# tturturiello/lightweight-snappy

Measured on AMD Instinct MI355X. Metric: compress + decompress MB/s at 1/2/4/8 MI355X; % HBM roofline; ratio vs ref, higher is better.
Workload: dtype u8

## Files before the change

### lightweight-snappy_amd/csrc/snappy_k2_emit.inc

```
    __shared__ __attribute__((aligned(16))) uint8_t stage_[kK2Stage + 4 + 4 * 64 + 16];
    auto *const stage = (__attribute__((address_space(3))) uint8_t *)stage_;
    const uint32_t lane = threadIdx.x;
    const uint32_t u = blockIdx.x;
    const uint32_t nt = ntok[u];
#if K2_RECORDS
    const uint64_t base = 0;
    const uint32_t L = rec.L;
#else
    const uint64_t base = (uint64_t)u * unit;
    const uint32_t L = (uint32_t)((n - base) < unit ? (n - base) : unit);
#endif
    const uint8_t *src = in + base;
    uint8_t *dst = out + offsets[u];
#if K2_RECORDS
    const uint32_t *tok = rec.tok, *tok_full = rec.tok_full;
#else
    const uint32_t *tok = reinterpret_cast<const uint32_t *>(tokens) + (uint64_t)u * tok_cap;
    const uint32_t *tok_full = reinterpret_cast<const uint32_t *>(tokens) + ((uint64_t)gridDim.x + u) * tok_cap;
#endif
    if (blockIdx.y == 0) {
        if (hdr_mode == SNAPPY_HDR_EVERY_UNIT) varint_put(L, dst, lane);
        else if (hdr_mode == SNAPPY_HDR_FIRST_UNIT && (K2_RECORDS || u == 0)) varint_put(header_value, dst, lane);
    }
    uint32_t kwn[kK2Per];
    auto load_kw = [&](uint32_t c, uint32_t *k) {
#pragma unroll
        for (uint32_t i = 0; i < kK2Per; i++) {
            const uint32_t t = c + kK2Per * lane + i;
            k[i] = tok[t < nt ? t : 0u];
        }
    };
    auto load_se = [&](uint32_t sg) {
#if K2_RECORDS
        return *reinterpret_cast<const uint2 *>(rec.segu + 2 * (sg * kK2Seg <= nt ? sg : 0u));
#else
        return *reinterpret_cast<const uint2 *>(seg_off + 2 * ((uint64_t)u * segs + (sg * kK2Seg <= nt ? sg : 0u)));
#endif
    };
    if (blockIdx.y * kK2Seg <= nt) load_kw(blockIdx.y * kK2Seg, kwn);
    uint2 sen = load_se(blockIdx.y);
    for (uint32_t sg = blockIdx.y; sg * kK2Seg <= nt; sg += gridDim.y) {
    const uint2 se = sen;
    sen = load_se(sg + gridDim.y);
    uint32_t o = se.x, carry = se.y;
    for (uint32_t c = sg * kK2Seg; c < (sg + 1) * kK2Seg && c <= nt; c += kK2Pass) {

    uint32_t gap[kK2Per], len[kK2Per], off[kK2Per], pe[kK2Per], litn[kK2Per], hl[kK2Per], sz[kK2Per];
    bool live[kK2Per];
    uint32_t lspan = 0;
    uint32_t kw[kK2Per];
#pragma unroll
    for (uint32_t i = 0; i < kK2Per; i++) kw[i] = kwn[i];
    {
        uint32_t cn = c + kK2Pass;
        if (!(cn < (sg + 1) * kK2Seg && cn <= nt)) cn = (sg + gridDim.y) * kK2Seg;
        if (cn <= nt) load_kw(cn, kwn);
    }
#pragma unroll
    for (uint32_t i = 0; i < kK2Per; i++) {
        const uint32_t t = c + kK2Per * lane + i;
        const bool has = t < nt;
        live[i] = t <= nt;
        const uint32_t k = has ? kw[i] : 0xFFFFFFFFu;
        const uint32_t lc = (k >> 16) & 0xFF, gc = k >> 24;
        off[i] = has ? k & 0xFFFF : 0u;
        gap[i] = has ? gc : 0u;
        len[i] = has ? lc + 4 : 0u;
        if (has && (lc == 255 || gc == 255)) {
            const uint32_t f = tok_full[t];
            gap[i] = f & 0xFFFF;
            len[i] = f >> 16;
        }
        lspan += gap[i] + len[i];
    }
    uint32_t span_tot;
    uint32_t cur = carry + wave_excl_scan(lspan, lane, &span_tot);
    uint32_t lsum = 0;
#pragma unroll
    for (uint32_t i = 0; i < kK2Per; i++) {
        const uint32_t t = c + kK2Per * lane + i;
        pe[i] = cur;
        litn[i] = t < nt ? gap[i] : (t == nt ? L - cur : 0u);
        cur += gap[i] + len[i];
        hl[i] = litn[i] ? (litn[i] <= 60 ? 1 : (litn[i] <= 256 ? 2 : 3)) : 0;
        sz[i] = hl[i] + litn[i] + ((live[i] && len[i]) ? copy_bytes(len[i], off[i]) : 0);
        lsum += sz[i];
    }
    uint32_t total;
    uint32_t rel = wave_excl_scan(lsum, lane, &total);
    const bool staged = total <= kK2Stage;
    const uint32_t sb = staged ? (uint32_t)(reinterpret_cast<uintptr_t>(dst + o) & 3) : 0u;
    uint64_t longs[kK2Per];
    uint32_t d0v[kK2Per];
    uint32_t lw[kK2Per][5], lsh[kK2Per];
    bool wide[kK2Per];
#pragma unroll
    for (uint32_t i = 0; i < kK2Per; i++) {
        wide[i] = base + pe[i] + 20 <= n;
        const bool ld = !SNAPPY_K2_NOLIT && staged && wide[i] && live[i] && litn[i] != 0 && litn[i] <= 16;
        const uintptr_t sa = reinterpret_cast<uintptr_t>(src + pe[i]);
        lsh[i] = (uint32_t)(sa & 3);
        const auto *aw = reinterpret_cast<const __attribute__((address_space(1))) uint32_t *>(
            ld ? sa - lsh[i] : reinterpret_cast<uintptr_t>(tok));
#pragma unroll
        for (uint32_t j = 0; j < 5; j++) lw[i][j] = aw[j];
    }
#pragma unroll
    for (uint32_t i = 0; i < kK2Per; i++) {
        const bool wide_ok = wide[i];
        if (staged) put_element_lds(stage, rel + sb, src, pe[i], litn[i], hl[i], len[i], off[i], wide_ok, live[i], lane,
                                    lw[i], lsh[i]);
        else if (live[i]) put_element(dst + o + rel, src, pe[i], litn[i], hl[i], len[i], off[i], wide_ok);
        longs[i] = __ballot(live[i] && litn[i] > 16);
        d0v[i] = rel + sb + hl[i];
        rel += sz[i];
    }
#pragma unroll
    for (uint32_t i = 0; i < kK2Per && !SNAPPY_K2_NOLIT; i++) {
        if (staged) k2_long_literals(stage, src, longs[i], litn[i], pe[i], d0v[i], lane);
        else k2_long_literals(dst + o, src, in + n, longs[i], litn[i], pe[i], d0v[i], lane);
    }
    if (staged) {
        __builtin_amdgcn_wave_barrier();
        uint8_t *g = dst + o;
        uint32_t head = (4 - sb) & 3;
        if (head > total) head = total;
        if (lane < head) g[lane] = stage[sb + lane];
        const uint32_t nw = (total - head) >> 2;
        uint32_t *gw = reinterpret_cast<uint32_t *>(g + head);
        const auto *sw = reinterpret_cast<const __attribute__((address_space(3))) uint32_t *>(stage + sb + head);
        for (uint32_t k = lane; k < nw; k += 64) gw[k] = sw[k];
        const uint32_t tail0 = head + 4 * nw;
        if (lane < total - tail0) g[tail0 + lane] = stage[sb + tail0 + lane];
    }
    __builtin_amdgcn_wave_barrier();
    o += total;
    carry += span_tot;
    }
    }
```

### lightweight-snappy_amd/csrc/snappy_kernels.hip

```cpp
#include <hip/hip_runtime.h>
#include <stdint.h>
#include <type_traits>

#include "snappy_kernels.h"

#ifndef SNAPPY_TU
#define SNAPPY_TU 0
#endif
#define SNAPPY_TU_COMPRESS (SNAPPY_TU != 2)
#define SNAPPY_TU_DECODE (SNAPPY_TU != 1)

#if ((defined(SNAPPY_K2_NOLIT) && SNAPPY_K2_NOLIT) || defined(SNAPPY_K4_NOFAR)) && !defined(SNAPPY_MEASUREMENT_BUILD)
#error "SNAPPY_K2_NOLIT / SNAPPY_K4_NOFAR write wrong output: measurement builds only (-DSNAPPY_MEASUREMENT_BUILD)"
#endif

namespace snappy_amd {

__device__ int amdgcn_writelane(int val, int lanesel, int old) __asm("llvm.amdgcn.writelane.i32");


constexpr uint32_t kTable = 4096;
constexpr uint32_t kMul = 0x1e35a7bdu;

typedef uint32_t u32x4 __attribute__((ext_vector_type(4)));
// ... 1249 lines not shown
    }
#endif
#ifdef SNAPPY_K1R_STATS
    if (!REC && lane == 0) {
        uint64_t *st = reinterpret_cast<uint64_t *>(tokens + (uint64_t)gridDim.x * tok_cap) + 4 * (uint64_t)u;
        st[0] = clock64() - t_loop;
#if defined(SNAPPY_K1R_LSTAMPS)
        st[1] = seg[0] | (seg[1] << 32);
        st[3] = seg[2] | (seg[3] << 32);
        st[2] = seg[4] | (seg[5] << 32);
#else
        st[1] = n_farc | ((uint64_t)n_reload << 32);
        st[2] = n_probe | ((uint64_t)n_round << 32);
        st[3] = n_match | ((uint64_t)n_refresh << 32);
#endif
    }
#endif
}

#if SNAPPY_TU_COMPRESS
__global__ __launch_bounds__(64, 3) void k1r_match_units(const uint8_t *__restrict__ in, uint64_t n, uint32_t unit,
                                                          uint32_t hdr_mode, uint64_t header_value,
                                                          uint2 *__restrict__ tokens, uint32_t tok_cap,
                                                          uint32_t *__restrict__ ntok_out,
                                                          uint32_t *__restrict__ sizes,
                                                          uint32_t *__restrict__ seg_off, uint32_t segs)
{
    k1r_body<false>(in, n, unit, hdr_mode, header_value, tokens, tok_cap, ntok_out, sizes, seg_off, segs);
}
#endif

#if SNAPPY_TU_COMPRESS
__global__ __launch_bounds__(64, 3) void k1r_match_units64(const uint8_t *__restrict__ in, uint64_t n, uint32_t unit,
                                                            uint32_t hdr_mode, uint64_t header_value,
                                                            uint2 *__restrict__ tokens, uint32_t tok_cap,
                                                            uint32_t *__restrict__ ntok_out,
                                                            uint32_t *__restrict__ sizes,
                                                            uint32_t *__restrict__ seg_off, uint32_t segs)
{
    k1r_body<true>(in, n, unit, hdr_mode, header_value, tokens, tok_cap, ntok_out, sizes, seg_off, segs);
}
#endif

__device__ __forceinline__ uint64_t rfl64(uint64_t v)
{
    return ((uint64_t)rfl((uint32_t)(v >> 32)) << 32) | rfl((uint32_t)v);
}

template <bool BIG>
__device__ __forceinline__ void kr1_record(const uint8_t *__restrict__ in, const uint64_t *__restrict__ off_len,
                                           const uint32_t *__restrict__ list, const uint64_t *__restrict__ sbase,
                                           uint32_t *__restrict__ scratch, uint32_t *__restrict__ ntok_out,
                                           uint32_t *__restrict__ sizes)
{
    K1Record rec;
    rec.u = rfl(list[blockIdx.x]);
    rec.L = rfl((uint32_t)off_len[2 * (uint64_t)rec.u + 1]);
    rec.src = in + rfl64(off_len[2 * (uint64_t)rec.u]);
    const uint32_t tok_cap = records_tok_cap(rec.L);
    rec.tok = scratch + rfl64(sbase[rec.u]);
    rec.tok_full = rec.tok + tok_cap;
    rec.segu = rec.tok_full + tok_cap;
    k1r_body<BIG, true>(nullptr, 0, 0, SNAPPY_HDR_EVERY_UNIT, 0, nullptr, 0, ntok_out, sizes, nullptr, 0, rec);
}

#if SNAPPY_TU_COMPRESS
__global__ __launch_bounds__(64, 3) void kr1_match_records(const uint8_t *__restrict__ in,
                                                            const uint64_t *__restrict__ off_len,
                                                            const uint32_t *__restrict__ list,
                                                            const uint64_t *__restrict__ sbase,
                                                            uint32_t *__restrict__ scratch,
                                                            uint32_t *__restrict__ ntok_out,
                                                            uint32_t *__restrict__ sizes)
{
    kr1_record<false>(in, off_len, list, sbase, scratch, ntok_out, sizes);
}

__global__ __launch_bounds__(64, 3) void kr1_match_records64(const uint8_t *__restrict__ in,
                                                              const uint64_t *__restrict__ off_len,
                                                              const uint32_t *__restrict__ list,
                                                              const uint64_t *__restrict__ sbase,
                                                              uint32_t *__restrict__ scratch,
                                                              uint32_t *__restrict__ ntok_out,
                                                              uint32_t *__restrict__ sizes)
{
    kr1_record<true>(in, off_len, list, sbase, scratch, ntok_out, sizes);
}
#endif

template <bool BIG>
__device__ __forceinline__ void kr1_lunit(const uint8_t *__restrict__ in, const uint64_t *__restrict__ off_len,
                                          const uint32_t *__restrict__ list, const uint32_t *__restrict__ urec,
                                          const uint64_t *__restrict__ ubase, const uint64_t *__restrict__ sbase,
                                          uint32_t *__restrict__ scratch, uint32_t *__restrict__ ntok_out,
                                          uint32_t *__restrict__ sizes)
{
    K1Record rec;
    rec.u = rfl(list[blockIdx.x]);
    const uint32_t r = rfl(urec[rec.u]);
    const uint32_t blk = rec.u - rfl((uint32_t)ubase[r]);
    const uint64_t len = rfl64(off_len[2 * (uint64_t)r + 1]);
    const uint64_t at = (uint64_t)blk * SNAPPY_BLOCK;
    rec.L = (uint32_t)(len - at < SNAPPY_BLOCK ? len - at : SNAPPY_BLOCK);
    rec.src = in + rfl64(off_len[2 * (uint64_t)r]) + at;
    const uint32_t tok_cap = records_tok_cap(rec.L);
    rec.tok = scratch + rfl64(sbase[rec.u]);
    rec.tok_full = rec.tok + tok_cap;
    rec.segu = rec.tok_full + tok_cap;
    k1r_body<BIG, true>(nullptr, 0, 0, blk == 0 ? SNAPPY_HDR_FIRST_UNIT : SNAPPY_HDR_NONE, len, nullptr, 0, ntok_out,
                        sizes, nullptr, 0, rec);
}

#if SNAPPY_TU_COMPRESS
__global__ __launch_bounds__(64, 3) void kr1_match_lunits(const uint8_t *__restrict__ in,
                                                           const uint64_t *__restrict__ off_len,
                                                           const uint32_t *__restrict__ list,
                                                           const uint32_t *__restrict__ urec,
                                                           const uint64_t *__restrict__ ubase,
                                                           const uint64_t *__restrict__ sbase,
                                                           uint32_t *__restrict__ scratch,
                                                           uint32_t *__restrict__ ntok_out,
                                                           uint32_t *__restrict__ sizes)
{
    kr1_lunit<false>(in, off_len, list, urec, ubase, sbase, scratch, ntok_out, sizes);
}

__global__ __launch_bounds__(64, 3) void kr1_match_lunits64(const uint8_t *__restrict__ in,
                                                             const uint64_t *__restrict__ off_len,
                                                             const uint32_t *__restrict__ list,
                                                             const uint32_t *__restrict__ urec,
                                                             const uint64_t *__restrict__ ubase,
                                                             const uint64_t *__restrict__ sbase,
                                                             uint32_t *__restrict__ scratch,
                                                             uint32_t *__restrict__ ntok_out,
                                                             uint32_t *__restrict__ sizes)
{
    kr1_lunit<true>(in, off_len, list, urec, ubase, sbase, scratch, ntok_out, sizes);
}
#endif

__device__ __forceinline__ uint32_t wave_excl_scan32(uint32_t v, uint32_t *total)
{
    uint32_t x = v;
    x += dpp0<0x111, 0xF>(x);
    x += dpp0<0x112, 0xF>(x);
    x += dpp0<0x114, 0xF>(x);
    x += dpp0<0x118, 0xF>(x);
    x += dpp0<0x142, 0xA>(x);
    *total = (uint32_t)__builtin_amdgcn_readlane((int)x, 31);
    return x - v;
}

template <typename P>
__device__ __forceinline__ void put_copy(P *o, uint32_t len, uint32_t off)
{
    while (len > 68) {
        o[0] = 0xFE; o[1] = (uint8_t)off; o[2] = (uint8_t)(off >> 8);
        o += 3; len -= 64;
    }
    if (len > 64) {
        o[0] = 0xEE; o[1] = (uint8_t)off; o[2] = (uint8_t)(off >> 8);
        o += 3; len -= 60;
    }
    if (len < 12 && off < 2048) {
        o[0] = (uint8_t)((((off >> 8) << 5) + ((len - 4) << 2) + 1));
        o[1] = (uint8_t)off;
    } else {
        o[0] = (uint8_t)(((len - 1) << 2) | 2); o[1] = (uint8_t)off; o[2] = (uint8_t)(off >> 8);
    }
}

template <typename P>
__device__ __forceinline__ void put_element(P *w, const uint8_t *__restrict__ src, uint32_t s0, uint32_t litn,
                                            uint32_t hl, uint32_t len, uint32_t off, bool wide_ok)
{
    if (hl == 1) w[0] = (uint8_t)((litn - 1) << 2);
    else if (hl == 2) { w[0] = 60 << 2; w[1] = (uint8_t)(litn - 1); }
    else if (hl == 3) { w[0] = 61 << 2; w[1] = (uint8_t)(litn - 1); w[2] = (uint8_t)((litn - 1) >> 8); }
    if (litn <= 16) {
        if (wide_ok) {
            const uintptr_t sa = reinterpret_cast<uintptr_t>(src + s0);
            const uint32_t sh = (uint32_t)(sa & 3);
            const uint32_t *aw = reinterpret_cast<const uint32_t *>(sa - sh);
            const uint32_t d0 = aw[0], d1 = aw[1], d2 = aw[2], d3 = aw[3], d4 = aw[4];
            const uint32_t r[4] = {__builtin_amdgcn_alignbyte(d1, d0, sh), __builtin_amdgcn_alignbyte(d2, d1, sh),
                                   __builtin_amdgcn_alignbyte(d3, d2, sh), __builtin_amdgcn_alignbyte(d4, d3, sh)};
#pragma unroll
            for (uint32_t j = 0; j < 16; j++)
                if (j < litn) w[hl + j] = (uint8_t)(r[j >> 2] >> (8 * (j & 3)));
        } else {
            for (uint32_t j = 0; j < litn; j++) w[hl + j] = src[s0 + j];
        }
    }
    if (len) put_copy(w + hl + litn, len, off);
}

#ifndef SNAPPY_K2_STAGE
#define SNAPPY_K2_STAGE 4096
#endif
constexpr uint32_t kK2Stage = SNAPPY_K2_STAGE;

__device__ __forceinline__ void put_element_lds(__attribute__((address_space(3))) uint8_t *stage, uint32_t at,
                                                const uint8_t *__restrict__ src, uint32_t s0, uint32_t litn,
                                                uint32_t hl, uint32_t len, uint32_t off, bool wide_ok, bool live,
                                                uint32_t lane, const uint32_t *lw, uint32_t sh)
{
    const uint32_t dum = kK2Stage + 4 + 4 * lane;
#define K2_ST8(cond, adr, v) stage[(cond) ? (adr) : dum] = (uint8_t)(v)
    const uint32_t lm1 = litn - 1;
    K2_ST8(live && hl >= 1, at, hl == 1 ? lm1 << 2 : (hl == 2 ? 60u << 2 : 61u << 2));
    K2_ST8(live && hl >= 2, at + 1, lm1);
    K2_ST8(live && hl == 3, at + 2, lm1 >> 8);
    const uint32_t lp = at + hl;
    if (litn <= 16) {
        if (wide_ok) {
            const uint32_t r0 = __builtin_amdgcn_alignbyte(lw[1], lw[0], sh), r1 = __builtin_amdgcn_alignbyte(lw[2], lw[1], sh);
            const uint32_t r2 = __builtin_amdgcn_alignbyte(lw[3], lw[2], sh), r3 = __builtin_amdgcn_alignbyte(lw[4], lw[3], sh);
#define K2_ST32(k, r) *(__attribute__((address_space(3))) u32u *)(stage + (live && 4 * (k) + 4 <= litn ? lp + 4 * (k) : dum)) = (r)
            K2_ST32(0, r0); K2_ST32(1, r1); K2_ST32(2, r2); K2_ST32(3, r3);
#undef K2_ST32
            const uint32_t fb = litn & ~3u, rem = litn & 3u;
            const uint32_t rt = fb == 0 ? r0 : (fb == 4 ? r1 : (fb == 8 ? r2 : r3));
            K2_ST8(live && rem > 0, lp + fb, rt);
            K2_ST8(live && rem > 1, lp + fb + 1, rt >> 8);
            K2_ST8(live && rem > 2, lp + fb + 2, rt >> 16);
        } else if (live) {
            for (uint32_t j = 0; j < litn; j++) stage[lp + j] = src[s0 + j];
        }
    }
    const uint32_t cp = lp + litn;
    if (len <= 64) {
        const bool c1 = len < 12 && off < 2048;
        const bool has = live && len != 0;
        K2_ST8(has, cp, c1 ? (((off >> 8) << 5) + ((len - 4) << 2) + 1) : (((len - 1) << 2) | 2));
        K2_ST8(has, cp + 1, off);
        K2_ST8(has && !c1, cp + 2, off >> 8);
    } else if (live) {
        put_copy(stage + cp, len, off);
    }
#undef K2_ST8
}

__device__ __forceinline__ void k2_long_literals(__attribute__((address_space(3))) uint8_t *w,
                                                 const uint8_t *__restrict__ src, uint64_t longs, uint32_t litn,
                                                 uint32_t s0v, uint32_t d0v, uint32_t lane)
{
    while (longs) {
        const uint32_t k = (uint32_t)__builtin_ctzll(longs);
        longs &= longs - 1;
        const uint32_t ln = __builtin_amdgcn_readlane(litn, k);
        const uint32_t s0 = __builtin_amdgcn_readlane(s0v, k);
        const uint32_t d0 = __builtin_amdgcn_readlane(d0v, k);
        for (uint32_t j0 = 0; j0 < ln; j0 += 512) {
            uint8_t v[8];
#pragma unroll
            for (uint32_t q = 0; q < 8; q++) {
                const uint32_t j = j0 + 64 * q + lane;
                v[q] = j < ln ? src[s0 + j] : 0;
            }
#pragma unroll
            for (uint32_t q = 0; q < 8; q++) {
                const uint32_t j = j0 + 64 * q + lane;
                if (j < ln) w[d0 + j] = v[q];
            }
        }
    }
}

__device__ __forceinline__ void k2_long_literals(uint8_t *w, const uint8_t *__restrict__ src,
                                                 const uint8_t *__restrict__ end, uint64_t longs, uint32_t litn,
                                                 uint32_t s0v, uint32_t d0v, uint32_t lane)
{
    while (longs) {
        const uint32_t k = (uint32_t)__builtin_ctzll(longs);
        longs &= longs - 1;
        const uint32_t ln = __builtin_amdgcn_readlane(litn, k);
        const uint8_t *s = src + __builtin_amdgcn_readlane(s0v, k);
        uint8_t *d = w + __builtin_amdgcn_readlane(d0v, k);
        uint32_t head = (uint32_t)((4 - (reinterpret_cast<uintptr_t>(d) & 3)) & 3);
        if (head > ln) head = ln;
        if (lane < head) d[lane] = s[lane];
        const uint32_t nw = (ln - head) >> 2;
        const uint8_t *sb = s + head;
        const uint32_t sh = (uint32_t)(reinterpret_cast<uintptr_t>(sb) & 3);
        const uint32_t *sa = reinterpret_cast<const uint32_t *>(sb - sh);
        uint32_t *dw = reinterpret_cast<uint32_t *>(d + head);
        for (uint32_t k0 = 0; k0 < nw; k0 += 256) {
            uint32_t lo[4], hi[4];
#pragma unroll
            for (uint32_t q = 0; q < 4; q++) {
                const uint32_t kk = k0 + 64 * q + lane;
                lo[q] = hi[q] = 0;
                if (kk < nw) {
                    lo[q] = sa[kk];
                    if (sh) {
                        const uint8_t *pb = reinterpret_cast<const uint8_t *>(sa + kk + 1);
                        if (pb + 4 <= end) hi[q] = sa[kk + 1];
                        else for (uint32_t t = 0; t < sh; t++) hi[q] |= (uint32_t)pb[t] << (8 * t);
                    }
                }
            }
#pragma unroll
            for (uint32_t q = 0; q < 4; q++) {
                const uint32_t kk = k0 + 64 * q + lane;
                if (kk < nw) dw[kk] = __builtin_amdgcn_alignbyte(hi[q], lo[q], sh);
            }
        }
        const uint32_t t0 = head + 4 * nw;
        if (lane < ln - t0) d[t0 + lane] = s[t0 + lane];
    }
}

#ifndef SNAPPY_K2_NOLIT
#define SNAPPY_K2_NOLIT 0
#endif
struct K2Record {
    uint32_t L;
    const uint32_t *tok, *tok_full, *segu;
};

#if SNAPPY_TU_COMPRESS
__global__ __launch_bounds__(64, 6) void k2_emit_units(const uint8_t *__restrict__ in, uint64_t n, uint32_t unit,
                                                    uint32_t hdr_mode, uint64_t header_value,
                                                    const uint2 *__restrict__ tokens, uint32_t tok_cap,
                                                    const uint32_t *__restrict__ ntok,
                                                    const uint32_t *__restrict__ seg_off, uint32_t segs,
                                                    const uint64_t *__restrict__ offsets, uint8_t *__restrict__ out)
{
#define K2_RECORDS 0
#include "snappy_k2_emit.inc"
#undef K2_RECORDS
}

__device__ __forceinline__ void kr2_emit_one(const uint8_t *in, const K2Record rec, const uint32_t *ntok,
                                             const uint64_t *offsets, uint8_t *out,
                                             const uint32_t hdr_mode = SNAPPY_HDR_EVERY_UNIT,
                                             const uint64_t header_value = 0)
{
    const uint64_t n = rec.L;
#define K2_RECORDS 1
#include "snappy_k2_emit.inc"
#undef K2_RECORDS
}

__global__ __launch_bounds__(64, 6) void kr2_emit_records(const uint8_t *__restrict__ base,
                                                          const uint64_t *__restrict__ off_len,
                                                          const int32_t *__restrict__ status,
                                                          const uint64_t *__restrict__ sbase,
                                                          const uint32_t *__restrict__ scratch,
                                                          const uint32_t *__restrict__ ntok,
                                                          const uint64_t *__restrict__ offsets,
                                                          uint8_t *__restrict__ out)
{
    const uint32_t r = blockIdx.x;
    const int32_t st = status[r];
    const uint64_t off = off_len[2 * (uint64_t)r], len = off_len[2 * (uint64_t)r + 1], sb = sbase[r];
    if (st < 0) return;
    K2Record rec;
    rec.L = rfl((uint32_t)len);
    if (rec.L == 0) {
        if (blockIdx.y == 0 && threadIdx.x == 0) out[offsets[r]] = 0;
        return;
    }
    const uint32_t tok_cap = records_tok_cap(rec.L);
    rec.tok = scratch + rfl64(sb);
    rec.tok_full = rec.tok + tok_cap;
    rec.segu = rec.tok_full + tok_cap;
    kr2_emit_one(base + rfl64(off), rec, ntok, offsets, out);
}

__global__ __launch_bounds__(64, 6) void kr2_emit_lunits(const uint8_t *__restrict__ base,
                                                         const uint64_t *__restrict__ off_len,
                                                         const uint32_t *__restrict__ urec,
                                                         const uint64_t *__restrict__ ubase,
                                                         const uint64_t *__restrict__ sbase,
                                                         const uint32_t *__restrict__ scratch,
                                                         const uint32_t *__restrict__ ntok,
                                                         const uint64_t *__restrict__ offsets,
                                                         uint8_t *__restrict__ out)
{
    const uint32_t u = blockIdx.x;
    const uint32_t r = rfl(urec[u]);
    const uint64_t sb = sbase[u];
    const uint64_t off = off_len[2 * (uint64_t)r], len = rfl64(off_len[2 * (uint64_t)r + 1]);
    const uint32_t blk = u - rfl((uint32_t)ubase[r]);
    if (len == 0) {
        if (blockIdx.y == 0 && threadIdx.x == 0) out[offsets[u]] = 0;
        return;
    }
    const uint64_t at = (uint64_t)blk * SNAPPY_BLOCK;
    K2Record rec;
    rec.L = (uint32_t)(len - at < SNAPPY_BLOCK ? len - at : SNAPPY_BLOCK);
    const uint32_t tok_cap = records_tok_cap(rec.L);
    rec.tok = scratch + rfl64(sb);
    rec.tok_full = rec.tok + tok_cap;
    rec.segu = rec.tok_full + tok_cap;
    kr2_emit_one(base + rfl64(off) + at, rec, ntok, offsets, out, blk == 0 ? SNAPPY_HDR_FIRST_UNIT : SNAPPY_HDR_NONE,
                 len);
}
#endif

constexpr uint32_t kScanPer = 8;
[[maybe_unused]] constexpr uint32_t kScanTile = 1024 * kScanPer;

#if SNAPPY_TU_COMPRESS
__global__ __launch_bounds__(1024) void k3_scan(const uint32_t *__restrict__ sizes, uint64_t count,
                                                uint64_t *__restrict__ offsets, uint64_t *__restrict__ total)
{
    __shared__ uint32_t tile[kScanTile + kScanTile / 32];
    __shared__ uint32_t wtot[16];
    const uint32_t t = threadIdx.x, lane = t & 63, w = t >> 6;
#define K3_AT(i) ((i) + ((i) >> 5))
    uint64_t carry = 0;
    for (uint64_t b = 0; b < count; b += kScanTile) {
        const uint32_t m = (uint32_t)(count - b < kScanTile ? count - b : kScanTile);
        for (uint32_t i = t; i < kScanTile; i += 1024) tile[K3_AT(i)] = i < m ? sizes[b + i] : 0u;
        __syncthreads();
        uint32_t v[kScanPer], s = 0;
#pragma unroll
        for (uint32_t k = 0; k < kScanPer; k++) {
            v[k] = tile[K3_AT(t * kScanPer + k)];
            s += v[k];
        }
        const uint32_t x = wave_incl_scan(s);
        if (lane == 63) wtot[w] = x;
        __syncthreads();
        if (w == 0) {
            const uint32_t y = lane < 16 ? wtot[lane] : 0u;
            const uint32_t z = wave_incl_scan(y);
            if (lane < 16) wtot[lane] = z - y;
        }
        __syncthreads();
        uint32_t run = wtot[w] + x - s;
#pragma unroll
        for (uint32_t k = 0; k < kScanPer; k++) {
            tile[K3_AT(t * kScanPer + k)] = run;
            run += v[k];
        }
        __syncthreads();
        for (uint32_t i = t; i < m; i += 1024) offsets[b + i] = carry + tile[K3_AT(i)];
        if (t == 1023) wtot[0] = run;
        __syncthreads();
        carry += wtot[0];
        __syncthreads();
    }
#undef K3_AT
    if (t == 0) {
        offsets[count] = carry;
        *total = carry;
    }
}

__global__ __launch_bounds__(64) void k3_scan_wave(const uint32_t *__restrict__ sizes, uint64_t count,
                                                  uint64_t *__restrict__ offsets, uint64_t *__restrict__ total)
{
    const uint32_t lane = threadIdx.x;
    uint64_t carry = 0;
    for (uint64_t b = 0; b < count; b += 64 * kScanPer) {
        uint32_t v[kScanPer], s = 0;
#pragma unroll
        for (uint32_t k = 0; k < kScanPer; k++) {
            const uint64_t i = b + kScanPer * lane + k;
            v[k] = i < count ? sizes[i] : 0u;
            s += v[k];
        }
        uint32_t tot;
        uint32_t run = wave_excl_scan(s, lane, &tot);
#pragma unroll
        for (uint32_t k = 0; k < kScanPer; k++) {
            const uint64_t i = b + kScanPer * lane + k;
            if (i < count) offsets[i] = carry + run;
            run += v[k];
        }
        carry += tot;
    }
    if (lane == 0) {
        offsets[count] = carry;
        *total = carry;
    }
}
#endif

constexpr uint64_t kIdxOffMask = (1ull << 40) - 1;
constexpr uint32_t kIdxSkipShift = 40;
constexpr int32_t kK4Tail = 3;

__device__ __forceinline__ uint32_t load_dw_guarded(const uint8_t *comp, uint64_t a, uint64_t lim)
{
    if (a + 4 <= lim) return __builtin_nontemporal_load(reinterpret_cast<const uint32_t *>(comp + a));
    uint32_t w = 0;
    for (uint32_t k = 0; k < 4; k++)
        if (a + k < lim) w |= (uint32_t)comp[a + k] << (8 * k);
    return w;
}

__device__ __forceinline__ uint32_t load_seg(const uint8_t *comp, uint64_t a0, uint64_t lim, uint32_t lane)
{
    if (a0 + 256 <= lim) return __builtin_nontemporal_load(reinterpret_cast<const uint32_t *>(comp + a0) + lane);
    return load_dw_guarded(comp, a0 + 4 * lane, lim);
}

__device__ __forceinline__ void k4_flush(const uint8_t *ob, uint32_t M, uint8_t *dst, uint32_t F, uint32_t T,
                                         uint32_t lane)
{
    if (T <= F) return;
    if ((reinterpret_cast<uintptr_t>(dst) & 15) == 0) {
        uint32_t a = (F + 15) & ~15u;
        if (a > T) a = T;
        if (F + lane < a) dst[F + lane] = ob[(F + lane) & M];
        const uint32_t e = T & ~15u;
#pragma unroll 1
        for (uint32_t x = a + 16 * lane; x < e; x += 1024)
            *reinterpret_cast<u32x4 *>(dst + x) = *reinterpret_cast<const u32x4 *>(ob + (x & M));
        const uint32_t t0 = e > a ? e : a;
        if (t0 + lane < T) dst[t0 + lane] = ob[(t0 + lane) & M];
    } else {
#pragma unroll 1
        for (uint32_t x = F + lane; x < T; x += 64) dst[x] = ob[x & M];
    }
}

#define K4_LIT_ATTR __noinline__
__device__ K4_LIT_ATTR void k4_literal_hbm(const uint8_t *lsrc, uint32_t kl, uint32_t kop, uint8_t *ob, uint32_t M,
                                               uint8_t *dst, uint32_t lane)
{
    uint8_t *const d = dst + kop;
    const uint32_t h0 = (uint32_t)(-(uintptr_t)d & 3);
    const uint32_t h = h0 < kl ? h0 : kl;
    if (lane < h) d[lane] = lsrc[lane];
    const uint32_t nd = (kl - h) >> 2;
    const uint8_t *const s = lsrc + h;
    const uint32_t sa = (uint32_t)((uintptr_t)s & 3);
    const uint32_t *const s4 = reinterpret_cast<const uint32_t *>(s - sa);
    uint32_t *const d4 = reinterpret_cast<uint32_t *>(d + h);
#pragma unroll 1
    for (uint32_t i = lane; i < nd; i += 256) {
        uint32_t w[4];
#pragma unroll
        for (int m = 0; m < 4; m++) {
            const uint32_t j = i + 64 * m;
            w[m] = 0;
            if (j < nd) {
                const uint32_t lo = __builtin_nontemporal_load(s4 + j);
                w[m] = sa ? __builtin_amdgcn_alignbit(__builtin_nontemporal_load(s4 + j + 1), lo, 8 * sa) : lo;
            }
        }
#pragma unroll
        for (int m = 0; m < 4; m++)
            if (i + 64 * m < nd) d4[i + 64 * m] = w[m];
// ... 1544 lines not shown
```

Measured before the change: 80240.

## Restructure k2 emit to cut VGPR pressure and raise wave occupancy

Rewrites the k2 emit pass so each element is kept as two packed registers (literal length, plus len/offset) instead of many per-element arrays. Sizes and positions are recomputed on the fly, and addressing uses 32-bit offsets from scalar bases made uniform with readfirstlane. The staged and unstaged paths are split into separate branches, and long-literal handling becomes a non-unrolled loop using opaque asm copies. Launch bounds rise to 8 (units) and 7 (records) waves per EU. The aim is lower register use and better latency hiding, at the cost of extra recomputation and possible spills if the register budget is not met.

New measurement: 80530, median of 6. About the same (+0.4%).

```diff
diff --git a/lightweight-snappy_amd/csrc/snappy_k2_emit.inc b/lightweight-snappy_amd/csrc/snappy_k2_emit.inc
--- a/lightweight-snappy_amd/csrc/snappy_k2_emit.inc
+++ b/lightweight-snappy_amd/csrc/snappy_k2_emit.inc
@@ -11,9 +11,11 @@
     const uint32_t L = (uint32_t)((n - base) < unit ? (n - base) : unit);
 #endif
     const uint8_t *src = in + base;
+    const uint32_t s3 = (uint32_t)(reinterpret_cast<uintptr_t>(src) & 3);
+    const uint32_t room = (uint32_t)(n - base < 0x7FFFFFFFu ? n - base : 0x7FFFFFFFu);
     uint8_t *dst = out + offsets[u];
 #if K2_RECORDS
-    const uint32_t *tok = rec.tok, *tok_full = rec.tok_full;
+    const uint32_t *tok = rec.tok;
 #else
     const uint32_t *tok = reinterpret_cast<const uint32_t *>(tokens) + (uint64_t)u * tok_cap;
     const uint32_t *tok_full = reinterpret_cast<const uint32_t *>(tokens) + ((uint64_t)gridDim.x + u) * tok_cap;
@@ -22,31 +24,72 @@
         if (hdr_mode == SNAPPY_HDR_EVERY_UNIT) varint_put(L, dst, lane);
         else if (hdr_mode == SNAPPY_HDR_FIRST_UNIT && (K2_RECORDS || u == 0)) varint_put(header_value, dst, lane);
     }
+    uint32_t dst_lo = (uint32_t)reinterpret_cast<uintptr_t>(dst), dst_hi = (uint32_t)(reinterpret_cast<uintptr_t>(dst) >> 32);
+    asm volatile("" : "+v"(dst_lo), "+v"(dst_hi));
     uint32_t kwn[kK2Per];
     auto load_kw = [&](uint32_t c, uint32_t *k) {
 #pragma unroll
         for (uint32_t i = 0; i < kK2Per; i++) {
             const uint32_t t = c + kK2Per * lane + i;
-            k[i] = tok[t < nt ? t : 0u];
+            k[i] = *reinterpret_cast<const uint32_t *>(reinterpret_cast<const uint8_t *>(tok) + 4 * (t < nt ? t : 0u));
         }
     };
+#if K2_RECORDS
+    const uint8_t *const segp = reinterpret_cast<const uint8_t *>(tok) + 4 * rec.seg_at;
+#else
+    const uint8_t *const segp = reinterpret_cast<const uint8_t *>(seg_off + 2 * (uint64_t)u * segs);
+#endif
     auto load_se = [&](uint32_t sg) {
-#if K2_RECORDS
-        return *reinterpret_cast<const uint2 *>(rec.segu + 2 * (sg * kK2Seg <= nt ? sg : 0u));
-#else
-        return *reinterpret_cast<const uint2 *>(seg_off + 2 * ((uint64_t)u * segs + (sg * kK2Seg <= nt ? sg : 0u)));
-#endif
+        uint32_t at = 8 * (sg * kK2Seg <= nt ? sg : 0u);
+        asm volatile("" : "+v"(at));
+        return *reinterpret_cast<const uint2 *>(segp + at);
+    };
+#define K2_COLD_LANE(v) uint32_t v = lane; asm volatile("" : "+v"(v))
+#define K2_LONG_LITERALS(at0, COPY)                                                                   \
+    do {                                                                                              \
+        uint32_t s0v[kK2Per], d0v[kK2Per];                                                            \
+        uint32_t cur = pe0, at = (at0);                                                               \
+        _Pragma("unroll") for (uint32_t i = 0; i < kK2Per; i++) {                                     \
+            s0v[i] = cur;                                                                             \
+            d0v[i] = at + hdr_len(litn[i]);                                                           \
+            cur += litn[i] + (lo[i] >> 16);                                                           \
+            at += elem_size(litn[i], lo[i]);                                                          \
+        }                                                                                             \
+        K2_COLD_LANE(lane_c);                                                                         \
+        _Pragma("nounroll") for (uint32_t i = 0; i < kK2Per; i++) {                                   \
+            uint32_t vl = 0, vs = 0, vd = 0;                                                          \
+            _Pragma("unroll") for (uint32_t j = 0; j < kK2Per; j++)                                   \
+                if (j == i) {                                                                         \
+                    vl = litn[j];                                                                     \
+                    vs = s0v[j];                                                                      \
+                    vd = d0v[j];                                                                      \
+                }                                                                                     \
+            for (uint64_t m = __ballot(vl != 0 && !short_lit(vl, vs)); m; m &= m - 1) {               \
+                const uint32_t k = (uint32_t)__builtin_ctzll(m);                                      \
+                const uint32_t ln = __builtin_amdgcn_readlane(vl, k);                                 \
+                const uint32_t s0 = __builtin_amdgcn_readlane(vs, k);                                 \
+                const uint32_t d0 = __builtin_amdgcn_readlane(vd, k);                                 \
+                COPY;                                                                                 \
+            }                                                                                         \
+        }                                                                                             \
+    } while (0)
+    auto short_lit = [&](uint32_t ln, uint32_t at) -> bool { return ln - 1 < 16 && at + 20 <= room; };
+    auto hdr_len = [](uint32_t ln) -> uint32_t { return ln ? (ln <= 60 ? 1u : (ln <= 256 ? 2u : 3u)) : 0u; };
+    auto elem_size = [&](uint32_t ln, uint32_t lk) -> uint32_t {
+        return hdr_len(ln) + ln + (lk ? copy_bytes(lk >> 16, lk & 0xFFFF) : 0u);
     };
     if (blockIdx.y * kK2Seg <= nt) load_kw(blockIdx.y * kK2Seg, kwn);
     uint2 sen = load_se(blockIdx.y);
     for (uint32_t sg = blockIdx.y; sg * kK2Seg <= nt; sg += gridDim.y) {
     const uint2 se = sen;
     sen = load_se(sg + gridDim.y);
-    uint32_t o = se.x, carry = se.y;
+    uint8_t *g = reinterpret_cast<uint8_t *>((uint64_t)(uint32_t)__builtin_amdgcn_readfirstlane(dst_lo) |
+                                             (uint64_t)(uint32_t)__builtin_amdgcn_readfirstlane(dst_hi) << 32) +
+                 (uint32_t)__builtin_amdgcn_readfirstlane(se.x);
+    uint32_t carry = (uint32_t)__builtin_amdgcn_readfirstlane(se.y);
     for (uint32_t c = sg * kK2Seg; c < (sg + 1) * kK2Seg && c <= nt; c += kK2Pass) {
 
-    uint32_t gap[kK2Per], len[kK2Per], off[kK2Per], pe[kK2Per], litn[kK2Per], hl[kK2Per], sz[kK2Per];
-    bool live[kK2Per];
+    uint32_t litn[kK2Per], lo[kK2Per];
     uint32_t lspan = 0;
     uint32_t kw[kK2Per];
 #pragma unroll
@@ -60,81 +103,90 @@
     for (uint32_t i = 0; i < kK2Per; i++) {
         const uint32_t t = c + kK2Per * lane + i;
         const bool has = t < nt;
-        live[i] = t <= nt;
-        const uint32_t k = has ? kw[i] : 0xFFFFFFFFu;
+        const uint32_t k = kw[i];
         const uint32_t lc = (k >> 16) & 0xFF, gc = k >> 24;
-        off[i] = has ? k & 0xFFFF : 0u;
-        gap[i] = has ? gc : 0u;
-        len[i] = has ? lc + 4 : 0u;
+        uint32_t gp = gc, lk = ((lc + 4) << 16) | (k & 0xFFFF);
         if (has && (lc == 255 || gc == 255)) {
-            const uint32_t f = tok_full[t];
-            gap[i] = f & 0xFFFF;
-            len[i] = f >> 16;
+#if K2_RECORDS
+            const uint32_t f = *reinterpret_cast<const uint32_t *>(reinterpret_cast<const uint8_t *>(tok) + 4 * (rec.full_at + t));
+#else
+            const uint32_t f = *reinterpret_cast<const uint32_t *>(reinterpret_cast<const uint8_t *>(tok_full) + 4 * t);
+#endif
+            gp = f & 0xFFFF;
+            lk = (f & 0xFFFF0000u) | (k & 0xFFFF);
         }
-        lspan += gap[i] + len[i];
+        litn[i] = has ? gp : 0u;
+        lo[i] = has ? lk : 0u;
+        lspan += litn[i] + (lo[i] >> 16);
     }
     uint32_t span_tot;
-    uint32_t cur = carry + wave_excl_scan(lspan, lane, &span_tot);
+    const uint32_t pe0 = carry + wave_excl_scan(lspan, lane, &span_tot);
     uint32_t lsum = 0;
+    {
+        uint32_t cur = pe0;
 #pragma unroll
-    for (uint32_t i = 0; i < kK2Per; i++) {
-        const uint32_t t = c + kK2Per * lane + i;
-        pe[i] = cur;
-        litn[i] = t < nt ? gap[i] : (t == nt ? L - cur : 0u);
-        cur += gap[i] + len[i];
-        hl[i] = litn[i] ? (litn[i] <= 60 ? 1 : (litn[i] <= 256 ? 2 : 3)) : 0;
-        sz[i] = hl[i] + litn[i] + ((live[i] && len[i]) ? copy_bytes(len[i], off[i]) : 0);
-        lsum += sz[i];
+        for (uint32_t i = 0; i < kK2Per; i++) {
+            if (c + kK2Per * lane + i == nt) litn[i] = L - cur;
+            lsum += elem_size(litn[i], lo[i]);
+            cur += litn[i] + (lo[i] >> 16);
+        }
     }
     uint32_t total;
-    uint32_t rel = wave_excl_scan(lsum, lane, &total);
-    const bool staged = total <= kK2Stage;
-    const uint32_t sb = staged ? (uint32_t)(reinterpret_cast<uintptr_t>(dst + o) & 3) : 0u;
-    uint64_t longs[kK2Per];
-    uint32_t d0v[kK2Per];
-    uint32_t lw[kK2Per][5], lsh[kK2Per];
-    bool wide[kK2Per];
+    const uint32_t rel = wave_excl_scan(lsum, lane, &total);
+    if (total <= kK2Stage) {
+        const uint32_t sb = (uint32_t)(reinterpret_cast<uintptr_t>(g) & 3);
+        uint32_t lw[kK2Per][5];
+        {
+            const uint8_t *la = room >= 20 ? src - s3 : reinterpret_cast<const uint8_t *>(tok);
+            uint32_t cur = pe0;
 #pragma unroll
-    for (uint32_t i = 0; i < kK2Per; i++) {
-        wide[i] = base + pe[i] + 20 <= n;
-        const bool ld = !SNAPPY_K2_NOLIT && staged && wide[i] && live[i] && litn[i] != 0 && litn[i] <= 16;
-        const uintptr_t sa = reinterpret_cast<uintptr_t>(src + pe[i]);
-        lsh[i] = (uint32_t)(sa & 3);
-        const auto *aw = reinterpret_cast<const __attribute__((address_space(1))) uint32_t *>(
-            ld ? sa - lsh[i] : reinterpret_cast<uintptr_t>(tok));
+            for (uint32_t i = 0; i < kK2Per; i++) {
+                const bool ld = !SNAPPY_K2_NOLIT && short_lit(litn[i], cur);
+                const uint32_t ai = ld ? (s3 + cur) & ~3u : 0u;
 #pragma unroll
-        for (uint32_t j = 0; j < 5; j++) lw[i][j] = aw[j];
-    }
+                for (uint32_t j = 0; j < 5; j++) lw[i][j] = *reinterpret_cast<const uint32_t *>(la + ai + 4 * j);
+                cur += litn[i] + (lo[i] >> 16);
+            }
+        }
+        {
+            uint32_t cur = pe0, at = rel + sb;
 #pragma unroll
-    for (uint32_t i = 0; i < kK2Per; i++) {
-        const bool wide_ok = wide[i];
-        if (staged) put_element_lds(stage, rel + sb, src, pe[i], litn[i], hl[i], len[i], off[i], wide_ok, live[i], lane,
-                                    lw[i], lsh[i]);
-        else if (live[i]) put_element(dst + o + rel, src, pe[i], litn[i], hl[i], len[i], off[i], wide_ok);
-        longs[i] = __ballot(live[i] && litn[i] > 16);
-        d0v[i] = rel + sb + hl[i];
-        rel += sz[i];
-    }
-#pragma unroll
-    for (uint32_t i = 0; i < kK2Per && !SNAPPY_K2_NOLIT; i++) {
-        if (staged) k2_long_literals(stage, src, longs[i], litn[i], pe[i], d0v[i], lane);
-        else k2_long_literals(dst + o, src, in + n, longs[i], litn[i], pe[i], d0v[i], lane);
-    }
-    if (staged) {
+            for (uint32_t i = 0; i < kK2Per; i++) {
+                put_element_lds(stage, at, litn[i], hdr_len(litn[i]), lo[i] >> 16, lo[i] & 0xFFFF,
+                                short_lit(litn[i], cur), true, lane, lw[i], (s3 + cur) & 3);
+                cur += litn[i] + (lo[i] >> 16);
+                at += elem_size(litn[i], lo[i]);
+            }
+        }
+        if (!SNAPPY_K2_NOLIT) K2_LONG_LITERALS(rel + sb, k2_long_literal(stage, src, ln, s0, d0, lane_c));
         __builtin_amdgcn_wave_barrier();
-        uint8_t *g = dst + o;
         uint32_t head = (4 - sb) & 3;
         if (head > total) head = total;
         if (lane < head) g[lane] = stage[sb + lane];
         const uint32_t nw = (total - head) >> 2;
-        uint32_t *gw = reinterpret_cast<uint32_t *>(g + head);
-        const auto *sw = reinterpret_cast<const __attribute__((address_space(3))) uint32_t *>(stage + sb + head);
-        for (uint32_t k = lane; k < nw; k += 64) gw[k] = sw[k];
+        for (uint32_t b = 4 * lane; b < 4 * nw; b += 256)
+            *reinterpret_cast<uint32_t *>(g + head + b) =
+                *reinterpret_cast<const __attribute__((address_space(3))) uint32_t *>(stage + sb + head + b);
         const uint32_t tail0 = head + 4 * nw;
         if (lane < total - tail0) g[tail0 + lane] = stage[sb + tail0 + lane];
+    } else {
+        {
+            uint32_t cur = pe0, at = rel;
+#pragma unroll
+            for (uint32_t i = 0; i < kK2Per; i++) {
+                if (litn[i] | lo[i])
+                    put_element(g, at, src, cur, litn[i], hdr_len(litn[i]), lo[i] >> 16, lo[i] & 0xFFFF,
+                                short_lit(litn[i], cur));
+                cur += litn[i] + (lo[i] >> 16);
+                at += elem_size(litn[i], lo[i]);
+            }
+        }
+        if (!SNAPPY_K2_NOLIT) K2_LONG_LITERALS(rel, k2_long_literal(g, src, room, ln, s0, d0, lane_c));
     }
     __builtin_amdgcn_wave_barrier();
-    o += total;
+    g += total;
     carry += span_tot;
     }
     }
+#undef K2_LONG_LITERALS
+#undef K2_COLD_LANE
diff --git a/lightweight-snappy_amd/csrc/snappy_kernels.hip b/lightweight-snappy_amd/csrc/snappy_kernels.hip
--- a/lightweight-snappy_amd/csrc/snappy_kernels.hip
+++ b/lightweight-snappy_amd/csrc/snappy_kernels.hip
@@ -1425,47 +1425,45 @@
 }
 
 template <typename P>
-__device__ __forceinline__ void put_copy(P *o, uint32_t len, uint32_t off)
+__device__ __forceinline__ void put_copy(P *o, uint32_t at, uint32_t len, uint32_t off)
 {
     while (len > 68) {
-        o[0] = 0xFE; o[1] = (uint8_t)off; o[2] = (uint8_t)(off >> 8);
-        o += 3; len -= 64;
+        o[at] = 0xFE; o[at + 1] = (uint8_t)off; o[at + 2] = (uint8_t)(off >> 8);
+        at += 3; len -= 64;
     }
     if (len > 64) {
-        o[0] = 0xEE; o[1] = (uint8_t)off; o[2] = (uint8_t)(off >> 8);
-        o += 3; len -= 60;
+        o[at] = 0xEE; o[at + 1] = (uint8_t)off; o[at + 2] = (uint8_t)(off >> 8);
+        at += 3; len -= 60;
     }
     if (len < 12 && off < 2048) {
-        o[0] = (uint8_t)((((off >> 8) << 5) + ((len - 4) << 2) + 1));
-        o[1] = (uint8_t)off;
+        o[at] = (uint8_t)((((off >> 8) << 5) + ((len - 4) << 2) + 1));
+        o[at + 1] = (uint8_t)off;
     } else {
-        o[0] = (uint8_t)(((len - 1) << 2) | 2); o[1] = (uint8_t)off; o[2] = (uint8_t)(off >> 8);
+        o[at] = (uint8_t)(((len - 1) << 2) | 2); o[at + 1] = (uint8_t)off; o[at + 2] = (uint8_t)(off >> 8);
     }
 }
 
 template <typename P>
-__device__ __forceinline__ void put_element(P *w, const uint8_t *__restrict__ src, uint32_t s0, uint32_t litn,
-                                            uint32_t hl, uint32_t len, uint32_t off, bool wide_ok)
-{
-    if (hl == 1) w[0] = (uint8_t)((litn - 1) << 2);
-    else if (hl == 2) { w[0] = 60 << 2; w[1] = (uint8_t)(litn - 1); }
-    else if (hl == 3) { w[0] = 61 << 2; w[1] = (uint8_t)(litn - 1); w[2] = (uint8_t)((litn - 1) >> 8); }
-    if (litn <= 16) {
-        if (wide_ok) {
-            const uintptr_t sa = reinterpret_cast<uintptr_t>(src + s0);
-            const uint32_t sh = (uint32_t)(sa & 3);
-            const uint32_t *aw = reinterpret_cast<const uint32_t *>(sa - sh);
-            const uint32_t d0 = aw[0], d1 = aw[1], d2 = aw[2], d3 = aw[3], d4 = aw[4];
-            const uint32_t r[4] = {__builtin_amdgcn_alignbyte(d1, d0, sh), __builtin_amdgcn_alignbyte(d2, d1, sh),
-                                   __builtin_amdgcn_alignbyte(d3, d2, sh), __builtin_amdgcn_alignbyte(d4, d3, sh)};
+__device__ __forceinline__ void put_element(P *w, uint32_t at, const uint8_t *__restrict__ src, uint32_t s0,
+                                            uint32_t litn, uint32_t hl, uint32_t len, uint32_t off, bool short_lit)
+{
+    if (hl == 1) w[at] = (uint8_t)((litn - 1) << 2);
+    else if (hl == 2) { w[at] = 60 << 2; w[at + 1] = (uint8_t)(litn - 1); }
+    else if (hl == 3) { w[at] = 61 << 2; w[at + 1] = (uint8_t)(litn - 1); w[at + 2] = (uint8_t)((litn - 1) >> 8); }
+    if (short_lit) {
+        const uint32_t s3 = (uint32_t)(reinterpret_cast<uintptr_t>(src) & 3);
+        const uint32_t sh = (s3 + s0) & 3, ai = (s3 + s0) & ~3u;
+        const uint8_t *sa = src - s3;
+        uint32_t d[5];
 #pragma unroll
-            for (uint32_t j = 0; j < 16; j++)
-                if (j < litn) w[hl + j] = (uint8_t)(r[j >> 2] >> (8 * (j & 3)));
-        } else {
-            for (uint32_t j = 0; j < litn; j++) w[hl + j] = src[s0 + j];
-        }
-    }
-    if (len) put_copy(w + hl + litn, len, off);
+        for (uint32_t j = 0; j < 5; j++) d[j] = *reinterpret_cast<const uint32_t *>(sa + ai + 4 * j);
+        const uint32_t r[4] = {__builtin_amdgcn_alignbyte(d[1], d[0], sh), __builtin_amdgcn_alignbyte(d[2], d[1], sh),
+                               __builtin_amdgcn_alignbyte(d[3], d[2], sh), __builtin_amdgcn_alignbyte(d[4], d[3], sh)};
+#pragma unroll
+        for (uint32_t j = 0; j < 16; j++)
+            if (j < litn) w[at + hl + j] = (uint8_t)(r[j >> 2] >> (8 * (j & 3)));
+    }
+    if (len) put_copy(w, at + hl + litn, len, off);
 }
 
 #ifndef SNAPPY_K2_STAGE
@@ -1474,9 +1472,9 @@
 constexpr uint32_t kK2Stage = SNAPPY_K2_STAGE;
 
 __device__ __forceinline__ void put_element_lds(__attribute__((address_space(3))) uint8_t *stage, uint32_t at,
-                                                const uint8_t *__restrict__ src, uint32_t s0, uint32_t litn,
-                                                uint32_t hl, uint32_t len, uint32_t off, bool wide_ok, bool live,
-                                                uint32_t lane, const uint32_t *lw, uint32_t sh)
+                                                uint32_t litn, uint32_t hl, uint32_t len, uint32_t off,
+                                                bool short_lit, bool live, uint32_t lane, const uint32_t *lw,
+                                                uint32_t sh)
 {
     const uint32_t dum = kK2Stage + 4 + 4 * lane;
 #define K2_ST8(cond, adr, v) stage[(cond) ? (adr) : dum] = (uint8_t)(v)
@@ -1485,21 +1483,18 @@
     K2_ST8(live && hl >= 2, at + 1, lm1);
     K2_ST8(live && hl == 3, at + 2, lm1 >> 8);
     const uint32_t lp = at + hl;
-    if (litn <= 16) {
-        if (wide_ok) {
-            const uint32_t r0 = __builtin_amdgcn_alignbyte(lw[1], lw[0], sh), r1 = __builtin_amdgcn_alignbyte(lw[2], lw[1], sh);
-            const uint32_t r2 = __builtin_amdgcn_alignbyte(lw[3], lw[2], sh), r3 = __builtin_amdgcn_alignbyte(lw[4], lw[3], sh);
-#define K2_ST32(k, r) *(__attribute__((address_space(3))) u32u *)(stage + (live && 4 * (k) + 4 <= litn ? lp + 4 * (k) : dum)) = (r)
-            K2_ST32(0, r0); K2_ST32(1, r1); K2_ST32(2, r2); K2_ST32(3, r3);
+    {
+        const uint32_t sl = short_lit ? litn : 0u;
+        const uint32_t r0 = __builtin_amdgcn_alignbyte(lw[1], lw[0], sh), r1 = __builtin_amdgcn_alignbyte(lw[2], lw[1], sh);
+        const uint32_t r2 = __builtin_amdgcn_alignbyte(lw[3], lw[2], sh), r3 = __builtin_amdgcn_alignbyte(lw[4], lw[3], sh);
+#define K2_ST32(k, r) *(__attribute__((address_space(3))) u32u *)(stage + (live && 4 * (k) + 4 <= sl ? lp + 4 * (k) : dum)) = (r)
+        K2_ST32(0, r0); K2_ST32(1, r1); K2_ST32(2, r2); K2_ST32(3, r3);
 #undef K2_ST32
-            const uint32_t fb = litn & ~3u, rem = litn & 3u;
-            const uint32_t rt = fb == 0 ? r0 : (fb == 4 ? r1 : (fb == 8 ? r2 : r3));
-            K2_ST8(live && rem > 0, lp + fb, rt);
-            K2_ST8(live && rem > 1, lp + fb + 1, rt >> 8);
-            K2_ST8(live && rem > 2, lp + fb + 2, rt >> 16);
-        } else if (live) {
-            for (uint32_t j = 0; j < litn; j++) stage[lp + j] = src[s0 + j];
-        }
+        const uint32_t fb = sl & ~3u, rem = sl & 3u;
+        const uint32_t rt = fb == 0 ? r0 : (fb == 4 ? r1 : (fb == 8 ? r2 : r3));
+        K2_ST8(live && rem > 0, lp + fb, rt);
+        K2_ST8(live && rem > 1, lp + fb + 1, rt >> 8);
+        K2_ST8(live && rem > 2, lp + fb + 2, rt >> 16);
     }
     const uint32_t cp = lp + litn;
     if (len <= 64) {
@@ -1509,91 +1504,81 @@
         K2_ST8(has, cp + 1, off);
         K2_ST8(has && !c1, cp + 2, off >> 8);
     } else if (live) {
-        put_copy(stage + cp, len, off);
+        put_copy(stage, cp, len, off);
     }
 #undef K2_ST8
 }
 
-__device__ __forceinline__ void k2_long_literals(__attribute__((address_space(3))) uint8_t *w,
-                                                 const uint8_t *__restrict__ src, uint64_t longs, uint32_t litn,
-                                                 uint32_t s0v, uint32_t d0v, uint32_t lane)
-{
-    while (longs) {
-        const uint32_t k = (uint32_t)__builtin_ctzll(longs);
-        longs &= longs - 1;
-        const uint32_t ln = __builtin_amdgcn_readlane(litn, k);
-        const uint32_t s0 = __builtin_amdgcn_readlane(s0v, k);
-        const uint32_t d0 = __builtin_amdgcn_readlane(d0v, k);
-        for (uint32_t j0 = 0; j0 < ln; j0 += 512) {
-            uint8_t v[8];
+__device__ __forceinline__ void k2_long_literal(__attribute__((address_space(3))) uint8_t *w,
+                                                const uint8_t *__restrict__ src, uint32_t ln, uint32_t s0,
+                                                uint32_t d0, uint32_t lane)
+{
+    asm volatile("" : "+v"(ln), "+v"(s0), "+v"(d0));
+    for (uint32_t j0 = 0; j0 < ln; j0 += 512) {
+        uint8_t v[8];
 #pragma unroll
-            for (uint32_t q = 0; q < 8; q++) {
-                const uint32_t j = j0 + 64 * q + lane;
-                v[q] = j < ln ? src[s0 + j] : 0;
+        for (uint32_t q = 0; q < 8; q++) {
+            const uint32_t j = j0 + 64 * q + lane;
+            v[q] = j < ln ? src[s0 + j] : 0;
+        }
+#pragma unroll
+        for (uint32_t q = 0; q < 8; q++) {
+            const uint32_t j = j0 + 64 * q + lane;
+            if (j < ln) w[d0 + j] = v[q];
+        }
+    }
+}
+
+__device__ __forceinline__ void k2_long_literal(uint8_t *w, const uint8_t *__restrict__ src, uint32_t room,
+                                                uint32_t ln, uint32_t s0, uint32_t d0, uint32_t lane)
+{
+    asm volatile("" : "+v"(ln), "+v"(s0), "+v"(d0));
+    uint32_t head = (4 - ((uint32_t)reinterpret_cast<uintptr_t>(w) + d0)) & 3;
+    if (head > ln) head = ln;
+    if (lane < head) w[d0 + lane] = src[s0 + lane];
+    const uint32_t s3 = (uint32_t)(reinterpret_cast<uintptr_t>(src) & 3);
+    const uint8_t *sa = src - s3;
+    const uint32_t so = s3 + s0 + head, sh = so & 3, oa = so & ~3u;
+    uint32_t nw = (ln - head) >> 2;
+    if (sh) {
+        const uint32_t lim = room + s3;
+        const uint32_t safe = lim >= oa + 8 ? (lim - oa - 4) >> 2 : 0u;
+        if (nw > safe) nw = safe;
+    }
+    const uint32_t dd = d0 + head;
+    for (uint32_t b0 = 4 * lane; b0 < 4 * nw; b0 += 1024) {
+        uint32_t lo[4], hi[4];
+#pragma unroll
+        for (uint32_t q = 0; q < 4; q++) {
+            const uint32_t b = b0 + 256 * q;
+            lo[q] = hi[q] = 0;
+            if (b < 4 * nw) {
+                lo[q] = *reinterpret_cast<const uint32_t *>(sa + oa + b);
+                if (sh) hi[q] = *reinterpret_cast<const uint32_t *>(sa + oa + b + 4);
             }
+        }
 #pragma unroll
-            for (uint32_t q = 0; q < 8; q++) {
-                const uint32_t j = j0 + 64 * q + lane;
-                if (j < ln) w[d0 + j] = v[q];
-            }
-        }
-    }
-}
-
-__device__ __forceinline__ void k2_long_literals(uint8_t *w, const uint8_t *__restrict__ src,
-                                                 const uint8_t *__restrict__ end, uint64_t longs, uint32_t litn,
-                                                 uint32_t s0v, uint32_t d0v, uint32_t lane)
-{
-    while (longs) {
-        const uint32_t k = (uint32_t)__builtin_ctzll(longs);
-        longs &= longs - 1;
-        const uint32_t ln = __builtin_amdgcn_readlane(litn, k);
-        const uint8_t *s = src + __builtin_amdgcn_readlane(s0v, k);
-        uint8_t *d = w + __builtin_amdgcn_readlane(d0v, k);
-        uint32_t head = (uint32_t)((4 - (reinterpret_cast<uintptr_t>(d) & 3)) & 3);
-        if (head > ln) head = ln;
-        if (lane < head) d[lane] = s[lane];
-        const uint32_t nw = (ln - head) >> 2;
-        const uint8_t *sb = s + head;
-        const uint32_t sh = (uint32_t)(reinterpret_cast<uintptr_t>(sb) & 3);
-        const uint32_t *sa = reinterpret_cast<const uint32_t *>(sb - sh);
-        uint32_t *dw = reinterpret_cast<uint32_t *>(d + head);
-        for (uint32_t k0 = 0; k0 < nw; k0 += 256) {
-            uint32_t lo[4], hi[4];
-#pragma unroll
-            for (uint32_t q = 0; q < 4; q++) {
-                const uint32_t kk = k0 + 64 * q + lane;
-                lo[q] = hi[q] = 0;
-                if (kk < nw) {
-                    lo[q] = sa[kk];
-                    if (sh) {
-                        const uint8_t *pb = reinterpret_cast<const uint8_t *>(sa + kk + 1);
-                        if (pb + 4 <= end) hi[q] = sa[kk + 1];
-                        else for (uint32_t t = 0; t < sh; t++) hi[q] |= (uint32_t)pb[t] << (8 * t);
-                    }
-                }
-            }
-#pragma unroll
-            for (uint32_t q = 0; q < 4; q++) {
-                const uint32_t kk = k0 + 64 * q + lane;
-                if (kk < nw) dw[kk] = __builtin_amdgcn_alignbyte(hi[q], lo[q], sh);
-            }
-        }
-        const uint32_t t0 = head + 4 * nw;
-        if (lane < ln - t0) d[t0 + lane] = s[t0 + lane];
-    }
-}
-
+        for (uint32_t q = 0; q < 4; q++) {
+            const uint32_t b = b0 + 256 * q;
+            if (b < 4 * nw) *reinterpret_cast<uint32_t *>(w + dd + b) = __builtin_amdgcn_alignbyte(hi[q], lo[q], sh);
+        }
+    }
+    const uint32_t t0 = head + 4 * nw;
+    if (lane < ln - t0) w[d0 + t0 + lane] = src[s0 + t0 + lane];
+}
+
+constexpr uint32_t kK2Waves = 8, kK2RecWaves = 7;
 #ifndef SNAPPY_K2_NOLIT
 #define SNAPPY_K2_NOLIT 0
 #endif
 struct K2Record {
     uint32_t L;
-    const uint32_t *tok, *tok_full, *segu;
+    const uint32_t *tok;
+    uint32_t full_at, seg_at;
 };
 
 #if SNAPPY_TU_COMPRESS
-__global__ __launch_bounds__(64, 6) void k2_emit_units(const uint8_t *__restrict__ in, uint64_t n, uint32_t unit,
+__global__ __launch_bounds__(64, kK2Waves) void k2_emit_units(const uint8_t *__restrict__ in, uint64_t n, uint32_t unit,
                                                     uint32_t hdr_mode, uint64_t header_value,
                                                     const uint2 *__restrict__ tokens, uint32_t tok_cap,
                                                     const uint32_t *__restrict__ ntok,
@@ -1616,7 +1601,7 @@
 #undef K2_RECORDS
 }
 
-__global__ __launch_bounds__(64, 6) void kr2_emit_records(const uint8_t *__restrict__ base,
+__global__ __launch_bounds__(64, kK2RecWaves) void kr2_emit_records(const uint8_t *__restrict__ base,
                                                           const uint64_t *__restrict__ off_len,
                                                           const int32_t *__restrict__ status,
                                                           const uint64_t *__restrict__ sbase,
@@ -1637,12 +1622,12 @@
     }
     const uint32_t tok_cap = records_tok_cap(rec.L);
     rec.tok = scratch + rfl64(sb);
-    rec.tok_full = rec.tok + tok_cap;
-    rec.segu = rec.tok_full + tok_cap;
+    rec.full_at = tok_cap;
+    rec.seg_at = 2 * tok_cap;
     kr2_emit_one(base + rfl64(off), rec, ntok, offsets, out);
 }
 
-__global__ __launch_bounds__(64, 6) void kr2_emit_lunits(const uint8_t *__restrict__ base,
+__global__ __launch_bounds__(64, kK2RecWaves) void kr2_emit_lunits(const uint8_t *__restrict__ base,
                                                          const uint64_t *__restrict__ off_len,
                                                          const uint32_t *__restrict__ urec,
                                                          const uint64_t *__restrict__ ubase,
@@ -1666,8 +1651,8 @@
     rec.L = (uint32_t)(len - at < SNAPPY_BLOCK ? len - at : SNAPPY_BLOCK);
     const uint32_t tok_cap = records_tok_cap(rec.L);
     rec.tok = scratch + rfl64(sb);
-    rec.tok_full = rec.tok + tok_cap;
-    rec.segu = rec.tok_full + tok_cap;
+    rec.full_at = tok_cap;
+    rec.seg_at = 2 * tok_cap;
     kr2_emit_one(base + rfl64(off) + at, rec, ntok, offsets, out, blk == 0 ? SNAPPY_HDR_FIRST_UNIT : SNAPPY_HDR_NONE,
                  len);
 }
```
